# mrmod/h264decode

Hardware: AMD Instinct MI355X
Metric: 1080p Main CABAC frames/sec (higher is better)
Workload: dtype u8; 1 GPU; 1920x1080 Main CABAC IPPP GOP-30, 256 independent streams per GPU (32 distinct, each used 8 times), QP 28, 1 slice/frame, 1 ref; parallelism=streams sharded, no collective

## Files before the change

### h264decode_amd/_lib.py

```python
import ctypes
import os
import re
import subprocess

_HERE = os.path.dirname(os.path.abspath(__file__))
_HEADER = os.path.join(_HERE, "..", "include", "h264mi.h")
_LIBPATH = os.environ.get("H264MI_LIB") or os.path.join(_HERE, "libh264mi.so")

_CT = {"int32_t": ctypes.c_int32, "uint32_t": ctypes.c_uint32, "int64_t": ctypes.c_int64, "uint64_t": ctypes.c_uint64, "uint8_t": ctypes.c_uint8,
       "double": ctypes.c_double, "float": ctypes.c_float, "void": None}


class H264MIError(RuntimeError):
    def __init__(self, code, msg):
        super().__init__("h264mi error %d: %s" % (code, msg))
        self.code = code


def _parse_structs():
    src = open(_HEADER).read()
    src = re.sub(r"/\*.*?\*/", "", src, flags=re.S)
    out = {}
    for body, name in re.findall(r"typedef struct \{(.*?)\}\s*(h264mi_\w+);", src, flags=re.S):
        fields = []
# ... 46 lines not shown
            raise H264MIError(-4, "libh264mi_hooks.so is not built (make -C h264decode_amd/csrc)")
        _hooks = ctypes.CDLL(path)
        I32 = ctypes.c_int32
        _hooks.h264mi_internal_dbprep_kernel_choice.argtypes = [I32, I32]
        _hooks.h264mi_internal_dbprep_kernel_choice.restype = I32
        _hooks.h264mi_internal_dbprep_check.argtypes = [ctypes.c_void_p, ctypes.POINTER(I32), ctypes.POINTER(I32), ctypes.POINTER(ctypes.c_int64)]
        _hooks.h264mi_internal_dbprep_check.restype = I32
        _hooks.h264mi_internal_set_dbprep_rows.argtypes = [ctypes.c_void_p, I32]
        _hooks.h264mi_internal_set_dbprep_rows.restype = I32
        _hooks.h264mi_internal_dbprep_ip_rows.argtypes = [I32, I32, I32]
        _hooks.h264mi_internal_dbprep_ip_rows.restype = I32
        _hooks.h264mi_internal_set_k5_waves.argtypes = [ctypes.c_void_p, I32]
        _hooks.h264mi_internal_set_k5_waves.restype = I32
        _hooks.h264mi_internal_deblock_edge_probe.argtypes = [I32, I32, I32] + [ctypes.c_void_p] * 6 + [ctypes.c_int64]
        _hooks.h264mi_internal_deblock_edge_probe.restype = I32
        _hooks.h264mi_internal_side_pending.argtypes = [ctypes.c_void_p, ctypes.POINTER(I32)]
        _hooks.h264mi_internal_side_pending.restype = I32
    return _hooks


def load():
    global _lib
    if _lib is not None:
        return _lib
    if not os.path.exists(_LIBPATH):
        raise H264MIError(-4, "libh264mi.so is not built (run h264decode_amd.build() / __graft_entry__.build()); "
                              "there is no CPU fallback for the decode path")
    L = ctypes.CDLL(_LIBPATH)
    P, I32, SZ = ctypes.POINTER, ctypes.c_int32, ctypes.c_size_t
    u8p, vp = ctypes.c_char_p, ctypes.c_void_p
# ... 111 lines not shown
```

### h264decode_amd/csrc/k_recon.hip

```cpp
#include <hip/hip_runtime.h>
#include <cstddef>
#include "mi_kernels.h"
#include "k_common.h"
#include "k_residual.h"

__device__ __forceinline__ int clip255(int v) { return min(max(v, 0), 255); }

struct ResBuf {
    int32_t tmp[384];
    int16_t luma[256];
    int16_t chroma[2][64];
    int32_t dc[24];
};

__device__ __forceinline__ void mb_residual(int lane, const MbRec *rec, const int16_t *coef, const ScalingSet *sc, ResBuf *rb) {
    const int type = rec->type, t8x8 = rec->t8x8, cbp = rec->cbp, qp = rec->qp;
    const int intra = MB_IS_INTRA(type), i16 = type == MBT_I16x16;
    const int cbp_l = cbp & 15, cbp_c = cbp >> 4;
    if (i16 && lane < 16) {
        const int i = lane >> 2, j = lane & 3;
        int acc = 0;
#pragma unroll
        for (int k = 0; k < 4; k++) {
            int aik = (i == 0) ? 1 : (i == 1 ? (k < 2 ? 1 : -1) : (i == 2 ? ((k == 0 || k == 3) ? 1 : -1) : ((k & 1) ? -1 : 1)));
            int rowsum = 0;
#pragma unroll
            for (int m = 0; m < 4; m++) {
                int amj = (j == 0) ? 1 : (j == 1 ? (m < 2 ? 1 : -1) : (j == 2 ? ((m == 0 || m == 3) ? 1 : -1) : ((m & 1) ? -1 : 1)));
// ... 93 lines not shown
        int16_t *dst = rb->chroma[c];
        dst[(y0 + 0) * 8 + x0] = static_cast<int16_t>((o0 + 32) >> 6);
        dst[(y0 + 1) * 8 + x0] = static_cast<int16_t>((o1 + 32) >> 6);
        dst[(y0 + 2) * 8 + x0] = static_cast<int16_t>((o2 + 32) >> 6);
        dst[(y0 + 3) * 8 + x0] = static_cast<int16_t>((o3 + 32) >> 6);
    }
    WAVE_SYNC();
}

__device__ __forceinline__ void zero_residual(int lane, ResBuf *rb) {
    for (int i = lane; i < 128; i += 64) reinterpret_cast<uint32_t *>(rb->luma)[i] = 0;
    reinterpret_cast<uint32_t *>(rb->chroma)[lane] = 0;
    WAVE_SYNC();
}

struct IntraWave {
    ResBuf rb;
    uint8_t tile[17][28];
    uint8_t tile_c[2][9][12];
    int16_t fe[2][32];
    MbRec rec;
    alignas(16) int16_t coef[MI_COEF_PER_MB];
};
#define MI_INTRA_MAX_ROWS 320
#define MI_INTRA_MAX_CHUNKS 8
struct IntraShared {
    IntraWave w[MI_INTRA_WAVES];
    ScalingSet sc;
    unsigned long long pend[MI_INTRA_MAX_ROWS][MI_INTRA_MAX_CHUNKS];
};

template <int N, typename FT, typename FL>
__device__ __forceinline__ int pred_dir(int mode, int x, int y, FT T, FL L) {
    switch (mode) {
    case 3: return (x == N - 1 && y == N - 1) ? (T(2 * N - 2) + 3 * T(2 * N - 1) + 2) >> 2 : (T(x + y) + 2 * T(x + y + 1) + T(x + y + 2) + 2) >> 2;
    case 4:
        if (x > y) return (T(x - y - 2) + 2 * T(x - y - 1) + T(x - y) + 2) >> 2;
        if (x < y) return (L(y - x - 2) + 2 * L(y - x - 1) + L(y - x) + 2) >> 2;
        return (T(0) + 2 * T(-1) + L(0) + 2) >> 2;
    case 5: {
        int z = 2 * x - y, k = x - (y >> 1);
        if (z < -1) return (L(y - 2 * x - 1) + 2 * L(y - 2 * x - 2) + L(y - 2 * x - 3) + 2) >> 2;
        if (z == -1) return (L(0) + 2 * T(-1) + T(0) + 2) >> 2;
// ... 9 lines not shown
    }
    case 7: {
        int k = x + (y >> 1);
        return !(y & 1) ? (T(k) + T(k + 1) + 1) >> 1 : (T(k) + 2 * T(k + 1) + T(k + 2) + 2) >> 2;
    }
    default: {
        int z = x + 2 * y, k = y + (x >> 1);
        if (z > 2 * N - 3) return L(N - 1);
        if (z == 2 * N - 3) return (L(N - 2) + 3 * L(N - 1) + 2) >> 2;
        if (!(z & 1)) return (L(k) + L(k + 1) + 1) >> 1;
        return (L(k) + 2 * L(k + 1) + L(k + 2) + 2) >> 2;
    }
    }
}

template <int N, typename FT, typename FL>
__device__ __forceinline__ void plane_params(FT T, FL L, int &a, int &b, int &c) {
    int hh = 0, vv = 0;
    constexpr int m = N / 2;
#pragma unroll
    for (int k = 1; k <= m; k++) {
        hh += k * (T(m - 1 + k) - T(m - 1 - k));
        vv += k * (L(m - 1 + k) - L(m - 1 - k));
    }
    a = 16 * (L(N - 1) + T(N - 1));
    b = N == 16 ? (5 * hh + 32) >> 6 : (34 * hh + 32) >> 6;
    c = N == 16 ? (5 * vv + 32) >> 6 : (34 * vv + 32) >> 6;
}

template <bool X>
__device__ __forceinline__ int ld_px(const g8 *p) {
    if (X) return static_cast<int>(__hip_atomic_load(p, __ATOMIC_RELAXED, __HIP_MEMORY_SCOPE_AGENT));
    return static_cast<int>(*p);
}
template <bool X>
__device__ __forceinline__ void st_px32(g8 *p, uint32_t v) {
    if (X)
        __hip_atomic_store(reinterpret_cast<g32 *>(p), v, __ATOMIC_RELAXED, __HIP_MEMORY_SCOPE_AGENT);
    else
        *reinterpret_cast<g32 *>(p) = v;
}
template <bool X>
__device__ __forceinline__ void st_px16(g8 *p, uint16_t v) {
    if (X)
        __hip_atomic_store(reinterpret_cast<g16 *>(p), v, __ATOMIC_RELAXED, __HIP_MEMORY_SCOPE_AGENT);
    else
        *reinterpret_cast<g16 *>(p) = v;
}

template <bool X>
__device__ void intra_mb(int lane, IntraWave *ws, const MbRec *rec, const int16_t *coef, const ScalingSet *sc, g8 *py, g8 *pcb, g8 *pcr, int W,
                         int mbx, int mby) {
    const int type = rec->type, av = rec->avail;
    const int a_left = av & MI_AV_LEFT, a_top = (av & MI_AV_TOP) != 0, a_tl = (av & MI_AV_TOPLEFT) != 0, a_tr = (av & MI_AV_TOPRIGHT) != 0;
    g8 *Y = py + static_cast<size_t>(mby * 16) * W + mbx * 16;
    const int Wc = W / 2;
    g8 *C0 = pcb + static_cast<size_t>(mby * 8) * Wc + mbx * 8, *C1 = pcr + static_cast<size_t>(mby * 8) * Wc + mbx * 8;
#define CPL(c) ((c) ? C1 : C0)
    if (type == MBT_NONE) {
        st_px32<X>(Y + static_cast<size_t>(lane >> 2) * W + (lane & 3) * 4, 0x80808080u);
        if (lane < 32) st_px32<X>(CPL(lane >> 4) + static_cast<size_t>((lane >> 1) & 7) * Wc + (lane & 1) * 4, 0x80808080u);
        return;
    }
    if (type == MBT_IPCM) {
        const uint8_t *pcm = reinterpret_cast<const uint8_t *>(coef);
        {
            int j = lane >> 2, i = (lane & 3) * 4;
// ... 13 lines not shown
        int y = lane - 32;
        ws->tile[y + 1][0] = a_left ? static_cast<uint8_t>(ld_px<X>(Y + static_cast<size_t>(y) * W - 1)) : static_cast<uint8_t>(128);
    }
    if (lane < 18) {
        int c = lane / 9, x = lane % 9 - 1;
        int ok = x < 0 ? a_tl : a_top;
        ws->tile_c[c][0][x + 1] = ok ? static_cast<uint8_t>(ld_px<X>(CPL(c) - static_cast<ptrdiff_t>(Wc) + x)) : static_cast<uint8_t>(128);
    } else if (lane >= 32 && lane < 48) {
        int c = (lane - 32) >> 3, y = lane & 7;
        ws->tile_c[c][y + 1][0] = a_left ? static_cast<uint8_t>(ld_px<X>(CPL(c) + static_cast<size_t>(y) * Wc - 1)) : static_cast<uint8_t>(128);
    }
    if ((rec->cbp & 0x3F) || type == MBT_I16x16)
        mb_residual(lane, rec, coef, sc, &ws->rb);
    else
        zero_residual(lane, &ws->rb);
    if (type == MBT_I16x16) {
        const int mode = rec->i16mode;
        auto T = [&](int x) { return static_cast<int>(ws->tile[0][x + 1]); };
        auto L = [&](int y) { return static_cast<int>(ws->tile[y + 1][0]); };
        const int j = lane >> 2, i0 = (lane & 3) * 4;
        int dc = 128, pa = 0, pb = 0, pc = 0;
        if (mode == 2) {
            int st = 0, sl = 0;
#pragma unroll
            for (int k = 0; k < 16; k++) st += T(k), sl += L(k);
            if (a_top && a_left)
                dc = (st + sl + 16) >> 5;
            else if (a_top)
                dc = (st + 8) >> 4;
            else if (a_left)
                dc = (sl + 8) >> 4;
        } else if (mode == 3)
            plane_params<16>(T, L, pa, pb, pc);
        uint32_t packed = 0;
#pragma unroll
        for (int k = 0; k < 4; k++) {
            int x = i0 + k, v;
            if (mode == 0)
                v = T(x);
            else if (mode == 1)
                v = L(j);
            else if (mode == 2)
                v = dc;
            else
                v = clip255((pa + pb * (x - 7) + pc * (j - 7) + 16) >> 5);
            v = clip255(v + ws->rb.luma[j * 16 + x]);
            packed |= static_cast<uint32_t>(v) << (8 * k);
        }
        st_px32<X>(Y + static_cast<size_t>(j) * W + i0, packed);
    } else if (type == MBT_I4x4) {
        for (int d = 0; d < 10; d++) {
            const int half = lane >> 4;
            const int by = (d >= 2 && d <= 7) ? (d & 1 ? (half ? 1 + ((d - 3) >> 1) : (d - 3) >> 1) : (half ? (d >> 1) : (d >> 1) - 1)) : (d < 2 ? 0 : 3);
            const int bx = d - 2 * by;
            const bool two = d >= 2 && d <= 7;
            if (lane < (two ? 32 : 16)) {
                const int mode = rec->ipm[by * 4 + bx];
                const int has_left = bx > 0 || a_left, has_top = by > 0 || a_top;
                int has_tr;
                if (by == 0)
                    has_tr = bx < 3 ? a_top : a_tr;
                else
                    has_tr = bx == 3 ? 0 : !((bx & 1) && (by & 1));
                const int x = lane & 3, y = (lane >> 2) & 3;
                const uint8_t *trow = &ws->tile[by * 4][bx * 4 + 1];
                auto T = [&](int k) { return static_cast<int>((k >= 4 && !has_tr) ? trow[3] : trow[k]); };
                auto L = [&](int k) { return k < 0 ? static_cast<int>(trow[-1]) : static_cast<int>(ws->tile[by * 4 + 1 + k][bx * 4]); };
                int v;
                if (mode == 0)
                    v = T(x);
                else if (mode == 1)
                    v = L(y);
                else if (mode == 2) {
                    int st = T(0) + T(1) + T(2) + T(3), sl = L(0) + L(1) + L(2) + L(3);
                    v = (has_top && has_left) ? (st + sl + 4) >> 3 : (has_top ? (st + 2) >> 2 : (has_left ? (sl + 2) >> 2 : 128));
                } else
                    v = pred_dir<4>(mode, x, y, T, L);
                v = clip255(v + ws->rb.luma[(by * 4 + y) * 16 + bx * 4 + x]);
                ws->tile[by * 4 + 1 + y][bx * 4 + 1 + x] = static_cast<uint8_t>(v);
            }
            WAVE_SYNC();
        }
    } else {
        for (int b8 = 0; b8 < 4; b8++) {
            const int x8 = b8 & 1, y8 = b8 >> 1;
            const int mode = rec->ipm[y8 * 8 + x8 * 2];
            const int has_left = x8 || a_left, has_top = y8 || a_top;
            const int has_tl = b8 == 0 ? a_tl : (b8 == 1 ? a_top : (b8 == 2 ? (a_left != 0) : 1));
            const int has_tr = b8 == 0 ? a_top : (b8 == 1 ? a_tr : (b8 == 2 ? 1 : 0));
            const uint8_t *trow = &ws->tile[y8 * 8][x8 * 8 + 1];
            auto Tr = [&](int k) { return k < 0 ? static_cast<int>(trow[-1]) : static_cast<int>((k >= 8 && !has_tr) ? trow[7] : trow[k]); };
            auto Lr = [&](int k) { return k < 0 ? static_cast<int>(trow[-1]) : static_cast<int>(ws->tile[y8 * 8 + 1 + k][x8 * 8]); };
            if (lane < 17) {
                int x = lane - 1, v;
                if (x < 0) {
                    if (has_top && has_left)
                        v = (Tr(0) + 2 * Tr(-1) + Lr(0) + 2) >> 2;
// ... 32 lines not shown
                    v = L(y);
                else if (mode == 2) {
                    int st = 0, sl = 0;
#pragma unroll
                    for (int k = 0; k < 8; k++) st += T(k), sl += L(k);
                    v = (has_top && has_left) ? (st + sl + 8) >> 4 : (has_top ? (st + 4) >> 3 : (has_left ? (sl + 4) >> 3 : 128));
                } else
                    v = pred_dir<8>(mode, x, y, T, L);
                v = clip255(v + ws->rb.luma[(y8 * 8 + y) * 16 + x8 * 8 + x]);
                WAVE_SYNC();
                ws->tile[y8 * 8 + 1 + y][x8 * 8 + 1 + x] = static_cast<uint8_t>(v);
            }
            WAVE_SYNC();
        }
    }
    if (type != MBT_I16x16) {
        const int j = lane >> 2, i0 = (lane & 3) * 4;
        const uint8_t *t = &ws->tile[j + 1][i0 + 1];
        uint32_t packed = t[0] | (t[1] << 8) | (t[2] << 16) | (static_cast<uint32_t>(t[3]) << 24);
        st_px32<X>(Y + static_cast<size_t>(j) * W + i0, packed);
    }
    {
        const int mode = rec->chroma_mode;
        const int c = lane >> 5, q = lane & 31, y = q >> 2, x0 = (q & 3) * 2;
        auto T = [&](int k) { return static_cast<int>(ws->tile_c[c][0][k + 1]); };
        auto L = [&](int k) { return static_cast<int>(ws->tile_c[c][k + 1][0]); };
        int pa = 0, pb = 0, pc = 0, dc = 128;
        if (mode == 3)
            plane_params<8>(T, L, pa, pb, pc);
        else if (mode == 0) {
            const int xo = x0 & 4, yo = y & 4;
            int st = T(xo) + T(xo + 1) + T(xo + 2) + T(xo + 3), sl = L(yo) + L(yo + 1) + L(yo + 2) + L(yo + 3);
            int use_t = a_top, use_l = a_left != 0;
            if (xo && !yo && a_top)
                use_l = 0;
            else if (!xo && yo && a_left)
                use_t = 0;
            if (use_t && use_l)
                dc = (st + sl + 4) >> 3;
            else if (use_t)
                dc = (st + 2) >> 2;
            else if (use_l)
                dc = (sl + 2) >> 2;
        }
        uint32_t packed = 0;
#pragma unroll
        for (int k = 0; k < 2; k++) {
            int x = x0 + k, v;
            if (mode == 0)
                v = dc;
            else if (mode == 1)
                v = L(y);
            else if (mode == 2)
                v = T(x);
            else
                v = clip255((pa + pb * (x - 3) + pc * (y - 3) + 16) >> 5);
            v = clip255(v + ws->rb.chroma[c][y * 8 + x]);
            packed |= static_cast<uint32_t>(v) << (8 * k);
        }
        st_px16<X>(CPL(c) + static_cast<size_t>(y) * Wc + x0, static_cast<uint16_t>(packed));
    }
}


struct IntraPic {
    int wmb, hmb, nchunks;
    int W;
    g8 *py, *pcb, *pcr;
    uint64_t mb_base;
    const MbRec *recs;
    __device__ __forceinline__ IntraPic(const PicDesc *pd, const DevTables *tab, const MbRec *mbrec, ScalingSet *sc, int tid, int nthreads) {
        wmb = static_cast<int>(pd->wmb), hmb = static_cast<int>(pd->hmb);
        W = static_cast<int>(pd->pitch);
        const PicPlace pp(pd);
        py = pp.base + pp.y, pcb = pp.base + pp.cb, pcr = pp.base + pp.cr;
        const uint32_t *src = reinterpret_cast<const uint32_t *>(&tab->scaling[pd->scaling_set]);
        for (int i = tid; i < static_cast<int>(sizeof(ScalingSet) / 4); i += nthreads) reinterpret_cast<uint32_t *>(sc)[i] = src[i];
        nchunks = (wmb + 63) >> 6;
        mb_base = pd->mb_base, recs = mbrec + mb_base;
    }
};

__device__ __forceinline__ unsigned long long intra_bits(const unsigned long long *mask, unsigned long long first, int n) {
    const unsigned long long w = first >> 6;
    const int sh = static_cast<int>(first & 63);
    unsigned long long m = mask[w] >> sh;
    if (sh) m |= mask[w + 1] << (64 - sh);
    return n >= 64 ? m : (m & ((1ull << n) - 1ull));
}

typedef unsigned long long IntraRows[MI_INTRA_MAX_ROWS][MI_INTRA_MAX_CHUNKS];

// ... 42 lines not shown
    if (ln < MI_COEF_BLOCKS) reinterpret_cast<uint4 *>(ws->coef)[2 * ln] = c0, reinterpret_cast<uint4 *>(ws->coef)[2 * ln + 1] = c1;
    WAVE_SYNC();
}

__device__ __forceinline__ void mb_done(IntraShared *sh, int mbx, int mby, int ln) {
    if (ln == 0) __hip_atomic_fetch_and(&sh->pend[mby][mbx >> 6], ~(1ull << (mbx & 63)), __ATOMIC_RELEASE, __HIP_MEMORY_SCOPE_WORKGROUP);
}

extern "C" __global__ void __launch_bounds__(MI_INTRA_WAVES * 64) k_intra(const uint32_t *pic_list, const PicDesc *pics, const FramePool *pools, const DevTables *tab,
                                                                          const MbRec *mbrec, const int16_t *coefs, const unsigned long long *intramask) {
    __shared__ IntraShared sh;
    __shared__ IntraRows s_intra;
    __shared__ uint32_t s_prefix[MI_INTRA_MAX_ROWS + 1];
    __shared__ uint32_t s_next;
    const int tid = static_cast<int>(threadIdx.x), lane = tid & 63, wave = tid >> 6;
    const IntraPic ip(&pics[pic_list[blockIdx.x]], tab, mbrec, &sh.sc, tid, MI_INTRA_WAVES * 64);
    const int wmb = ip.wmb, hmb = ip.hmb, nchunks = ip.nchunks;
    load_intra_masks(ip, intramask, &sh, s_intra, 0, hmb, tid, MI_INTRA_WAVES * 64);
    if (tid == 0) s_next = 0;
    __syncthreads();
    if (tid == 0) {
        uint32_t acc = 0;
        s_prefix[0] = 0;
        for (int r = 0; r < hmb; r++) {
            for (int c = 0; c < nchunks; c++) acc += static_cast<uint32_t>(__builtin_popcountll(s_intra[r][c]));
            s_prefix[r + 1] = acc;
        }
    }
    __syncthreads();
    IntraWave *ws = &sh.w[wave];
    const uint32_t n_intra = s_prefix[hmb];
// ... 27 lines not shown
                if (++chunk == nchunks) chunk = 0, row += MI_INTRA_WAVES;
                if (row >= hmb) break;
                mask = s_intra[row][chunk];
            }
            if (!mask) break;
            mbx = chunk * 64 + __ffsll(static_cast<long long>(mask)) - 1, mby = row;
            mask &= mask - 1;
        }
        mbx = __builtin_amdgcn_readfirstlane(mbx), mby = __builtin_amdgcn_readfirstlane(mby);
        int ln = lane;
        OPAQUE(ln);
        load_rec(ws, ip.recs + static_cast<uint64_t>(mby) * wmb + mbx, ln);
        if (sparse && mbx > 0) wait_mb(&sh, mbx - 1, mby);
        if (mby > 0) wait_row_above(&sh, mby, AboveSpan(mbx, wmb));
        gather_coefs(ws, coefs, ln);
        intra_mb<false>(ln, ws, &ws->rec, ws->coef, &sh.sc, ip.py, ip.pcb, ip.pcr, ip.W, mbx, mby);
        mb_done(&sh, mbx, mby, ln);
    }
}

extern "C" __global__ void __launch_bounds__(MI_INTRA_WAVES * 64) k_intra_x(const uint32_t *pic_list, const PicDesc *pics, const FramePool *pools, const DevTables *tab,
                                                                            const MbRec *mbrec, const int16_t *coefs, uint32_t *xdone_, uint32_t epoch, int nbands,
                                                                            uint32_t *ticket, uint32_t ticket_base, int wmb_max, uint32_t *xstatus, int wpr,
                                                                            const unsigned long long *intramask) {
    __shared__ IntraShared sh;
    __shared__ IntraRows s_intra;
    __shared__ uint32_t s_ticket;
    const int tid = static_cast<int>(threadIdx.x), lane = tid & 63, wave = tid >> 6, nthreads = static_cast<int>(blockDim.x), nwaves = nthreads >> 6;
    if (tid == 0) s_ticket = atomicAdd(ticket, 1u) - ticket_base;
    __syncthreads();
    const uint32_t tk = s_ticket, pic_i = tk / static_cast<uint32_t>(nbands);
    const int band = static_cast<int>(tk - pic_i * static_cast<uint32_t>(nbands));
    const PicDesc *pd = &pics[pic_list[pic_i]];
    const int wmb = static_cast<int>(pd->wmb), hmb = static_cast<int>(pd->hmb);
    const int r0 = band * hmb / nbands, r1 = (band + 1) * hmb / nbands;
    if (r0 >= r1) return;
    const IntraPic ip(pd, tab, mbrec, &sh.sc, tid, nthreads);
    const int nchunks = ip.nchunks;
    typedef __attribute__((address_space(1))) uint32_t gflag;
    int pband = band - 1;
    while (pband > 0 && pband * hmb / nbands == (pband + 1) * hmb / nbands) pband--;
    gflag *const xin = (gflag *)xdone_ + (static_cast<size_t>(pic_i) * nbands + (pband > 0 ? pband : 0)) * static_cast<size_t>(wmb_max);
    gflag *const xout = (gflag *)xdone_ + (static_cast<size_t>(pic_i) * nbands + band) * static_cast<size_t>(wmb_max);
    load_intra_masks(ip, intramask, &sh, s_intra, r0 > 0 ? r0 - 1 : 0, r1, tid, nthreads);
    __syncthreads();
    IntraWave *ws = &sh.w[wave];
    const int row_slot = wave / wpr, turn = wave - row_slot * wpr, row_slots = nwaves / wpr;
    for (int mby = r0 + row_slot; mby < r1; mby += row_slots) {
        const MbRec *row = ip.recs + static_cast<uint64_t>(mby) * wmb;
        const bool publish = mby == r1 - 1 && r1 < hmb;
        int nth = 0;
        for (int c = 0; c < nchunks; c++) {
// ... 16 lines not shown
                        const bool need = ln < 3 && col <= up.xr && ((sh.pend[mby - 1][col >> 6] >> (col & 63)) & 1ull);
                        const unsigned long long t_start = __builtin_amdgcn_s_memrealtime();
                        for (;;) {
                            const uint32_t v = need ? __hip_atomic_load(xin + col, __ATOMIC_RELAXED, __HIP_MEMORY_SCOPE_AGENT) : epoch;
                            if (__builtin_amdgcn_ballot_w64(v != epoch) == 0) break;
                            __builtin_amdgcn_s_sleep(2);
                            if (__builtin_amdgcn_s_memrealtime() - t_start > 400000000ull) {
                                if (ln == 0) atomicExch(xstatus, 0x3D000000u | static_cast<uint32_t>(mby));
                                break;
                            }
                        }
                        __builtin_amdgcn_fence(__ATOMIC_ACQUIRE, "wavefront");
                    }
                }
                gather_coefs(ws, coefs, ln);
                intra_mb<true>(ln, ws, &ws->rec, ws->coef, &sh.sc, ip.py, ip.pcb, ip.pcr, ip.W, mbx, mby);
                if (publish) {
                    asm volatile("s_waitcnt vmcnt(0)" ::: "memory");
                    if (ln == 0) __hip_atomic_store(xout + mbx, epoch, __ATOMIC_RELAXED, __HIP_MEMORY_SCOPE_AGENT);
                }
                mb_done(&sh, mbx, mby, ln);
            }
        }
    }
}
```

### h264decode_amd/csrc/mi_hooks.cpp

```cpp
#include <hip/hip_runtime.h>
#include <algorithm>
#include <cstdio>
#include <cstdlib>
#include <vector>
#include "mi_decoder.hpp"
#if defined(H264MI_TEST_HOOKS) && defined(__HIP__)
#include "k_deblock_edge.h"
#include "k_deblock_pk.h"
#endif

#if !defined(H264MI_TEST_HOOKS)
void hook_create_entropy(h264mi_decoder *, int *) {}
void hook_create_k5(h264mi_decoder *) {}
int hook_entropy_kernel(int chosen) { return chosen; }
int hook_dbprep_kernel(int chosen) { return chosen; }
void hook_after_sync(const h264mi_decoder *) {}
#else
void hook_create_entropy(h264mi_decoder *d, int *ent_cus) {
    if (const char *e = getenv("H264MI_ENT_LDS_PAD")) d->ent_lds_pad = static_cast<size_t>(atoi(e));
    if (const char *e = getenv("H264MI_ENT_CUS")) *ent_cus = atoi(e);
}
void hook_create_k5(h264mi_decoder *d) {
    if (const char *e = getenv("H264MI_K5_WAVES")) d->k5_max_waves = std::min(std::max(atoi(e), 1), MI_DEBLOCK8_MAX_WAVES);
}
// ... 261 lines not shown
    int nb = 1, nw = 1, ring = 1, b3 = 1, w3 = 1, roles = 1;
    mi_deblock_bands(n_pics, wmb, hmb, max_wgs, &nb, &nw, &ring, &roles);
    int wpr = 1;
    mi_intra_bands(n_pics, hmb, max_wgs, false, &b3, &w3, &wpr);
    *k5_bands = nb, *k5_waves = nw / roles, *k5_ring = ring, *k5_lds = static_cast<int64_t>(mi_deblock_lds_bytes_banded(nw, ring));
    *k3_bands = b3, *k3_waves = w3;
    return H264MI_OK;
}

extern "C" int32_t h264mi_internal_intra_plan(int32_t n_pics, int32_t hmb, int32_t max_wgs, int32_t p_only, int32_t band, int32_t *bands, int32_t *waves, int32_t *wpr, int32_t *row0) {
    if (!bands || !waves || !wpr || !row0 || n_pics < 1 || hmb < 1 || band < 0) return H264MI_EINVAL;
    int nb = 1, nw = 1, w = 1;
    mi_intra_bands(n_pics, hmb, max_wgs, p_only != 0, &nb, &nw, &w);
    *bands = nb, *waves = nw, *wpr = w, *row0 = band < nb ? band * hmb / nb : hmb;
    return H264MI_OK;
}

extern "C" int32_t h264mi_internal_set_epoch(h264mi_decoder *d, uint32_t v) {
    if (!d) return H264MI_EINVAL;
    GUARD(d);
    if (const int r = drain(d)) return r;
    d->x_epoch = d->x_tk5 = d->x_tk3 = v;
    HIP_TRY(hipMemcpy(d->d_xctl, &d->x_tk5, sizeof(uint32_t), hipMemcpyHostToDevice));
    HIP_TRY(hipMemcpy(d->d_xctl + 32, &d->x_tk3, sizeof(uint32_t), hipMemcpyHostToDevice));
    return H264MI_OK;
}

extern "C" int32_t h264mi_internal_dpb_trace(h264mi_decoder *d, int32_t stream, char *buf, size_t cap, size_t *len) {
    if (!d || !buf || !len || !cap || stream < 0 || stream >= static_cast<int>(d->st.size())) return H264MI_EINVAL;
    const Stage &g = d->stage[d->prep];
// ... 97 lines not shown
```

Measured before the change: 30350 frames/s.

## Rewrite intra prediction with lane-parallel DPP reductions and 4x4 pick table

Replaces the per-lane serial intra prediction (loops over edge samples for DC/plane, per-mode formulas) with cross-lane DPP/bpermute reductions for 16x16 and chroma DC/plane. It also adds a constexpr lookup table that maps each 4x4 mode/pixel to one of four precomputed edge vectors (edge, 3-tap, 2-tap, DC). Several 4x4 blocks are predicted in parallel along diagonals. The goal is to cut instruction count and divergence in the intra reconstruction kernel, at the cost of more LDS for the table and more complex lane shuffles. Test probes are added to check the new paths.

```diff
diff --git a/h264decode_amd/_lib.py b/h264decode_amd/_lib.py
--- a/h264decode_amd/_lib.py
+++ b/h264decode_amd/_lib.py
@@ -84,6 +84,10 @@
         _hooks.h264mi_internal_set_k5_waves.restype = I32
         _hooks.h264mi_internal_deblock_edge_probe.argtypes = [I32, I32, I32] + [ctypes.c_void_p] * 6 + [ctypes.c_int64]
         _hooks.h264mi_internal_deblock_edge_probe.restype = I32
+        _hooks.h264mi_internal_intra_pick_table.argtypes = [I32, ctypes.c_void_p, ctypes.c_int64]
+        _hooks.h264mi_internal_intra_pick_table.restype = I32
+        _hooks.h264mi_internal_intra_block_probe.argtypes = [I32] + [ctypes.c_void_p] * 5 + [ctypes.c_int64]
+        _hooks.h264mi_internal_intra_block_probe.restype = I32
         _hooks.h264mi_internal_side_pending.argtypes = [ctypes.c_void_p, ctypes.POINTER(I32)]
         _hooks.h264mi_internal_side_pending.restype = I32
     return _hooks
diff --git a/h264decode_amd/csrc/k_intra_pred.h b/h264decode_amd/csrc/k_intra_pred.h
--- /dev/null
+++ b/h264decode_amd/csrc/k_intra_pred.h
@@ -0,0 +1,239 @@
+#pragma once
+#include <hip/hip_runtime.h>
+#include <cstddef>
+#include <cstdint>
+#include "mi_kernels.h"
+#include "k_common.h"
+
+enum { IP_E = 0, IP_F3 = 1, IP_F2 = 2, IP_DC = 3 };
+#define IP4_LINE 13
+#define IP_BAD 0xFF
+constexpr uint8_t ip_pick(int vec, int idx) { return (idx < 0 || idx > 15) ? IP_BAD : static_cast<uint8_t>(idx << 2 | vec); }
+constexpr int ip4_t(int k) { return 5 + k; }
+constexpr int ip4_l(int k) { return 3 - k; }
+constexpr uint8_t ip4_tap3(int p, int q, int r) {
+    const int lo = p < r ? p : r, hi = p < r ? r : p;
+    const bool inner = lo == q - 1 && hi == q + 1, low_end = q == 0 && lo == 0 && hi == 1, high_end = q == IP4_LINE - 1 && lo == q - 1 && hi == q;
+    return (inner || low_end || high_end) ? ip_pick(IP_F3, q) : static_cast<uint8_t>(IP_BAD);
+}
+constexpr uint8_t ip4_tap2(int p, int q) { return (p - q == 1 || q - p == 1) ? ip_pick(IP_F2, p < q ? p : q) : static_cast<uint8_t>(IP_BAD); }
+constexpr uint8_t ip4_entry(int mode, int x, int y) {
+    switch (mode) {
+    case 0: return ip_pick(IP_E, ip4_t(x));
+    case 1: return ip_pick(IP_E, ip4_l(y));
+    case 2: return ip_pick(IP_DC, 0);
+    case 3: return (x == 3 && y == 3) ? ip4_tap3(ip4_t(6), ip4_t(7), ip4_t(7)) : ip4_tap3(ip4_t(x + y), ip4_t(x + y + 1), ip4_t(x + y + 2));
+    case 4:
+        if (x > y) return ip4_tap3(ip4_t(x - y - 2), ip4_t(x - y - 1), ip4_t(x - y));
+        if (x < y) return ip4_tap3(ip4_l(y - x - 2), ip4_l(y - x - 1), ip4_l(y - x));
+        return ip4_tap3(ip4_t(0), ip4_t(-1), ip4_l(0));
+    case 5: {
+        const int z = 2 * x - y, k = x - (y >> 1);
+        if (z < -1) return ip4_tap3(ip4_l(y - 2 * x - 1), ip4_l(y - 2 * x - 2), ip4_l(y - 2 * x - 3));
+        if (z == -1) return ip4_tap3(ip4_l(0), ip4_t(-1), ip4_t(0));
+        if (!(z & 1)) return ip4_tap2(ip4_t(k - 1), ip4_t(k));
+        return ip4_tap3(ip4_t(k - 2), ip4_t(k - 1), ip4_t(k));
+    }
+    case 6: {
+        const int z = 2 * y - x, k = y - (x >> 1);
+        if (z < -1) return ip4_tap3(ip4_t(x - 2 * y - 1), ip4_t(x - 2 * y - 2), ip4_t(x - 2 * y - 3));
+        if (z == -1) return ip4_tap3(ip4_l(0), ip4_t(-1), ip4_t(0));
+        if (!(z & 1)) return ip4_tap2(ip4_l(k - 1), ip4_l(k));
+        return ip4_tap3(ip4_l(k - 2), ip4_l(k - 1), ip4_l(k));
+    }
+    case 7: {
+        const int k = x + (y >> 1);
+        return !(y & 1) ? ip4_tap2(ip4_t(k), ip4_t(k + 1)) : ip4_tap3(ip4_t(k), ip4_t(k + 1), ip4_t(k + 2));
+    }
+    default: {
+        const int z = x + 2 * y, k = y + (x >> 1);
+        if (z > 5) return ip_pick(IP_E, ip4_l(3));
+        if (z == 5) return ip4_tap3(ip4_l(2), ip4_l(3), ip4_l(3));
+        if (!(z & 1)) return ip4_tap2(ip4_l(k), ip4_l(k + 1));
+        return ip4_tap3(ip4_l(k), ip4_l(k + 1), ip4_l(k + 2));
+    }
+    }
+}
+struct alignas(16) Ip4Table {
+    uint8_t e[9 * 16];
+};
+constexpr Ip4Table ip4_make_table() {
+    Ip4Table t{};
+    for (int m = 0; m < 9; m++)
+        for (int i = 0; i < 16; i++) t.e[m * 16 + i] = ip4_entry(m, i & 3, i >> 2);
+    return t;
+}
+constexpr bool ip4_table_ok(const Ip4Table &t) {
+    for (int i = 0; i < 9 * 16; i++)
+        if (t.e[i] == IP_BAD) return false;
+    return true;
+}
+constexpr Ip4Table ip4_table = ip4_make_table();
+static_assert(ip4_table_ok(ip4_table), "a formula of 8.3.1.2 that is no pick from E / F3 / F2 / DC");
+
+#if defined(__HIP__)
+static __constant__ Ip4Table ip4_table_dev = ip4_make_table();
+
+__device__ __forceinline__ int clip255(int v) { return min(max(v, 0), 255); }
+
+struct ResBuf {
+    int32_t tmp[384];
+    int16_t luma[256];
+    int16_t chroma[2][64];
+    int32_t dc[24];
+};
+#define IP_TILE_PITCH 28
+struct IntraWave {
+    ResBuf rb;
+    uint8_t tile[17][IP_TILE_PITCH];
+    uint8_t tile_c[2][9][12];
+    int16_t fe[2][32];
+    MbRec rec;
+    alignas(16) int16_t coef[MI_COEF_PER_MB];
+};
+
+template <bool X>
+__device__ __forceinline__ int ld_px(const g8 *p) {
+    if (X) return static_cast<int>(__hip_atomic_load(p, __ATOMIC_RELAXED, __HIP_MEMORY_SCOPE_AGENT));
+    return static_cast<int>(*p);
+}
+template <bool X>
+__device__ __forceinline__ void st_px32(g8 *p, uint32_t v) {
+    if (X)
+        __hip_atomic_store(reinterpret_cast<g32 *>(p), v, __ATOMIC_RELAXED, __HIP_MEMORY_SCOPE_AGENT);
+    else
+        *reinterpret_cast<g32 *>(p) = v;
+}
+template <bool X>
+__device__ __forceinline__ void st_px16(g8 *p, uint16_t v) {
+    if (X)
+        __hip_atomic_store(reinterpret_cast<g16 *>(p), v, __ATOMIC_RELAXED, __HIP_MEMORY_SCOPE_AGENT);
+    else
+        *reinterpret_cast<g16 *>(p) = v;
+}
+
+#define IP_DPP_QUAD_1032 0xB1
+#define IP_DPP_QUAD_2301 0x4E
+#define IP_DPP_ROW_SHL1 0x101
+#define IP_DPP_ROW_SHR1 0x111
+#define IP_DPP_ROW_ROR(n) (0x120 + (n))
+#define IP_DPP_HALF_MIRROR 0x141
+template <int CTRL>
+__device__ __forceinline__ int ip_row_nb(int v) { return __builtin_amdgcn_update_dpp(v, v, CTRL, 0xF, 0xF, false); }
+template <int CTRL>
+__device__ __forceinline__ int ip_dpp(int v) { return __builtin_amdgcn_update_dpp(0, v, CTRL, 0xF, 0xF, false); }
+__device__ __forceinline__ int ip_row_sum(int v) {
+    v += ip_dpp<IP_DPP_ROW_ROR(8)>(v);
+    v += ip_dpp<IP_DPP_ROW_ROR(4)>(v);
+    v += ip_dpp<IP_DPP_ROW_ROR(2)>(v);
+    v += ip_dpp<IP_DPP_ROW_ROR(1)>(v);
+    return v;
+}
+__device__ __forceinline__ int ip_quad_sum(int v) {
+    v += ip_dpp<IP_DPP_QUAD_1032>(v);
+    v += ip_dpp<IP_DPP_QUAD_2301>(v);
+    return v;
+}
+__device__ __forceinline__ int ip_lane_get(int v, int src_lane) { return __builtin_amdgcn_ds_bpermute(src_lane << 2, v); }
+
+__device__ __forceinline__ int ip4_sample(const uint8_t *corner, int lane, int pick, int res, int has_left, int has_top, int has_tr) {
+    const int l = lane & 15;
+    int k = min(l - 4, 8);
+    k = (k >= 5 && !has_tr) ? 4 : k;
+    const int e = corner[l < 4 ? (4 - l) * IP_TILE_PITCH : k];
+    const int below = ip_row_nb<IP_DPP_ROW_SHR1>(e), above = ip_row_nb<IP_DPP_ROW_SHL1>(e);
+    const int f3 = (below + 2 * e + above + 2) >> 2, f2 = (e + above + 1) >> 1;
+    const int s = ip_row_sum((l < 4 ? e : 0) | ((l >= 5 && l < 9) ? e << 16 : 0));
+    const int st = has_top ? s >> 16 : 0, sl = has_left ? s & 0xFFFF : 0, n = (has_top != 0) + (has_left != 0);
+    const int dc = n ? (st + sl + (1 << n)) >> (n + 1) : 128;
+    const uint32_t vecs = static_cast<uint32_t>(e) | static_cast<uint32_t>(f3) << 8 | static_cast<uint32_t>(f2) << 16 | static_cast<uint32_t>(dc) << 24;
+    const uint32_t got = static_cast<uint32_t>(__builtin_amdgcn_ds_bpermute(((lane & 0x30) << 2) | (pick & 0x3C), static_cast<int>(vecs)));
+    const int pred = static_cast<int>((got >> ((pick & 3) << 3)) & 255u);
+    return clip255(pred + res);
+}
+
+template <bool X>
+__device__ __forceinline__ void ip16_luma(int lane, const IntraWave *ws, int mode, int a_top, int a_left, g8 *Y, int W) {
+    const uint8_t *tile = &ws->tile[0][0];
+    const int j = lane >> 2, i0 = (lane & 3) * 4;
+    int p0, p1, p2, p3;
+    if (mode == 0) {
+        const uint32_t *row = reinterpret_cast<const uint32_t *>(tile + i0);
+        unpack4(__builtin_amdgcn_alignbyte(row[1], row[0], 1), p0, p1, p2, p3);
+    } else if (mode == 1)
+        p0 = p1 = p2 = p3 = tile[(j + 1) * IP_TILE_PITCH];
+    else {
+        const int r = lane & 31, i = r & 15, plane = mode == 3;
+        const int e = tile[(plane && i == 7) ? 0 : (r < 16 ? i + 1 : (i + 1) * IP_TILE_PITCH)];
+        const int s = ip_row_sum(plane ? (i == 7 ? -8 : i - 7) * e : e);
+        const int top = __builtin_amdgcn_readlane(s, 0), left = __builtin_amdgcn_readlane(s, 16);
+        if (!plane) {
+            int dc = 128;
+            if (a_top && a_left)
+                dc = (top + left + 16) >> 5;
+            else if (a_top)
+                dc = (top + 8) >> 4;
+            else if (a_left)
+                dc = (left + 8) >> 4;
+            p0 = p1 = p2 = p3 = dc;
+        } else {
+            const int a = 16 * (__builtin_amdgcn_readlane(e, 15) + __builtin_amdgcn_readlane(e, 31));
+            const int b = (5 * top + 32) >> 6, c = (5 * left + 32) >> 6;
+            const int base = a + b * (i0 - 7) + c * (j - 7) + 16;
+            p0 = clip255(base >> 5), p1 = clip255((base + b) >> 5), p2 = clip255((base + 2 * b) >> 5), p3 = clip255((base + 3 * b) >> 5);
+        }
+    }
+    const v2u rr = *reinterpret_cast<const v2u *>(&ws->rb.luma[j * 16 + i0]);
+    const int r0 = static_cast<int16_t>(rr.x & 0xFFFFu), r1 = static_cast<int>(rr.x) >> 16, r2 = static_cast<int16_t>(rr.y & 0xFFFFu), r3 = static_cast<int>(rr.y) >> 16;
+    st_px32<X>(Y + static_cast<size_t>(j) * W + i0, pack4(clip255(p0 + r0), clip255(p1 + r1), clip255(p2 + r2), clip255(p3 + r3)));
+}
+
+template <bool X>
+__device__ __forceinline__ void ip_tile_to_frame(int lane, const IntraWave *ws, g8 *Y, int W) {
+    const int j = lane >> 2, i0 = (lane & 3) * 4;
+    const uint32_t *row = reinterpret_cast<const uint32_t *>(&ws->tile[j + 1][i0]);
+    st_px32<X>(Y + static_cast<size_t>(j) * W + i0, __builtin_amdgcn_alignbyte(row[1], row[0], 1));
+}
+
+template <bool X>
+__device__ __forceinline__ void ip_chroma(int lane, const IntraWave *ws, int mode, int a_top, int a_left, g8 *C, int Wc) {
+    const int c = lane >> 5, q = lane & 31, y = q >> 2, x0 = (q & 3) * 2, first = lane & 32;
+    const uint8_t *tile = &ws->tile_c[c][0][0];
+    int p0, p1;
+    if (mode == 1)
+        p0 = p1 = tile[(y + 1) * 12];
+    else if (mode == 2)
+        p0 = tile[x0 + 1], p1 = tile[x0 + 2];
+    else {
+        const int i = q & 7, plane = mode == 3;
+        const int e = tile[(plane && i == 3) ? 0 : ((q & 8) ? (i + 1) * 12 : i + 1)];
+        if (!plane) {
+            const int s = ip_quad_sum(e), xo = x0 & 4, yo = y & 4;
+            const int st = ip_lane_get(s, first + xo), sl = ip_lane_get(s, first + 8 + yo);
+            int use_t = a_top, use_l = a_left != 0, dc = 128;
+            if (xo && !yo && a_top)
+                use_l = 0;
+            else if (!xo && yo && a_left)
+                use_t = 0;
+            if (use_t && use_l)
+                dc = (st + sl + 4) >> 3;
+            else if (use_t)
+                dc = (st + 2) >> 2;
+            else if (use_l)
+                dc = (sl + 2) >> 2;
+            p0 = p1 = dc;
+        } else {
+            int s = ip_quad_sum((i == 3 ? -4 : i - 3) * e);
+            s += ip_dpp<IP_DPP_HALF_MIRROR>(s);
+            const int hh = ip_lane_get(s, first), vv = ip_lane_get(s, first + 8);
+            const int a = 16 * (ip_lane_get(e, first + 7) + ip_lane_get(e, first + 15));
+            const int b = (34 * hh + 32) >> 6, cc = (34 * vv + 32) >> 6;
+            const int base = a + b * (x0 - 3) + cc * (y - 3) + 16;
+            p0 = clip255(base >> 5), p1 = clip255((base + b) >> 5);
+        }
+    }
+    const uint32_t rr = *reinterpret_cast<const uint32_t *>(&ws->rb.chroma[c][y * 8 + x0]);
+    const int r0 = static_cast<int16_t>(rr & 0xFFFFu), r1 = static_cast<int>(rr) >> 16;
+    st_px16<X>(C + static_cast<size_t>(y) * Wc + x0, static_cast<uint16_t>(clip255(p0 + r0) | clip255(p1 + r1) << 8));
+}
+#endif
diff --git a/h264decode_amd/csrc/k_recon.hip b/h264decode_amd/csrc/k_recon.hip
--- a/h264decode_amd/csrc/k_recon.hip
+++ b/h264decode_amd/csrc/k_recon.hip
@@ -3,15 +3,7 @@
 #include "mi_kernels.h"
 #include "k_common.h"
 #include "k_residual.h"
-
-__device__ __forceinline__ int clip255(int v) { return min(max(v, 0), 255); }
-
-struct ResBuf {
-    int32_t tmp[384];
-    int16_t luma[256];
-    int16_t chroma[2][64];
-    int32_t dc[24];
-};
+#include "k_intra_pred.h"
 
 __device__ __forceinline__ void mb_residual(int lane, const MbRec *rec, const int16_t *coef, const ScalingSet *sc, ResBuf *rb) {
     const int type = rec->type, t8x8 = rec->t8x8, cbp = rec->cbp, qp = rec->qp;
@@ -135,19 +127,12 @@
     WAVE_SYNC();
 }
 
-struct IntraWave {
-    ResBuf rb;
-    uint8_t tile[17][28];
-    uint8_t tile_c[2][9][12];
-    int16_t fe[2][32];
-    MbRec rec;
-    alignas(16) int16_t coef[MI_COEF_PER_MB];
-};
 #define MI_INTRA_MAX_ROWS 320
 #define MI_INTRA_MAX_CHUNKS 8
 struct IntraShared {
     IntraWave w[MI_INTRA_WAVES];
     ScalingSet sc;
+    Ip4Table pick4;
     unsigned long long pend[MI_INTRA_MAX_ROWS][MI_INTRA_MAX_CHUNKS];
 };
 
@@ -187,43 +172,9 @@
     }
 }
 
-template <int N, typename FT, typename FL>
-__device__ __forceinline__ void plane_params(FT T, FL L, int &a, int &b, int &c) {
-    int hh = 0, vv = 0;
-    constexpr int m = N / 2;
-#pragma unroll
-    for (int k = 1; k <= m; k++) {
-        hh += k * (T(m - 1 + k) - T(m - 1 - k));
-        vv += k * (L(m - 1 + k) - L(m - 1 - k));
-    }
-    a = 16 * (L(N - 1) + T(N - 1));
-    b = N == 16 ? (5 * hh + 32) >> 6 : (34 * hh + 32) >> 6;
-    c = N == 16 ? (5 * vv + 32) >> 6 : (34 * vv + 32) >> 6;
-}
-
 template <bool X>
-__device__ __forceinline__ int ld_px(const g8 *p) {
-    if (X) return static_cast<int>(__hip_atomic_load(p, __ATOMIC_RELAXED, __HIP_MEMORY_SCOPE_AGENT));
-    return static_cast<int>(*p);
-}
-template <bool X>
-__device__ __forceinline__ void st_px32(g8 *p, uint32_t v) {
-    if (X)
-        __hip_atomic_store(reinterpret_cast<g32 *>(p), v, __ATOMIC_RELAXED, __HIP_MEMORY_SCOPE_AGENT);
-    else
-        *reinterpret_cast<g32 *>(p) = v;
-}
-template <bool X>
-__device__ __forceinline__ void st_px16(g8 *p, uint16_t v) {
-    if (X)
-        __hip_atomic_store(reinterpret_cast<g16 *>(p), v, __ATOMIC_RELAXED, __HIP_MEMORY_SCOPE_AGENT);
-    else
-        *reinterpret_cast<g16 *>(p) = v;
-}
-
-template <bool X>
-__device__ void intra_mb(int lane, IntraWave *ws, const MbRec *rec, const int16_t *coef, const ScalingSet *sc, g8 *py, g8 *pcb, g8 *pcr, int W,
-                         int mbx, int mby) {
+__device__ void intra_mb(int lane, IntraWave *ws, const MbRec *rec, const int16_t *coef, const ScalingSet *sc, const Ip4Table *pk, g8 *py, g8 *pcb, g8 *pcr,
+                         int W, int mbx, int mby) {
     const int type = rec->type, av = rec->avail;
     const int a_left = av & MI_AV_LEFT, a_top = (av & MI_AV_TOP) != 0, a_tl = (av & MI_AV_TOPLEFT) != 0, a_tr = (av & MI_AV_TOPRIGHT) != 0;
     g8 *Y = py + static_cast<size_t>(mby * 16) * W + mbx * 16;
@@ -267,73 +218,34 @@
         mb_residual(lane, rec, coef, sc, &ws->rb);
     else
         zero_residual(lane, &ws->rb);
-    if (type == MBT_I16x16) {
-        const int mode = rec->i16mode;
-        auto T = [&](int x) { return static_cast<int>(ws->tile[0][x + 1]); };
-        auto L = [&](int y) { return static_cast<int>(ws->tile[y + 1][0]); };
-        const int j = lane >> 2, i0 = (lane & 3) * 4;
-        int dc = 128, pa = 0, pb = 0, pc = 0;
-        if (mode == 2) {
-            int st = 0, sl = 0;
-#pragma unroll
-            for (int k = 0; k < 16; k++) st += T(k), sl += L(k);
-            if (a_top && a_left)
-                dc = (st + sl + 16) >> 5;
-            else if (a_top)
-                dc = (st + 8) >> 4;
-            else if (a_left)
-                dc = (sl + 8) >> 4;
-        } else if (mode == 3)
-            plane_params<16>(T, L, pa, pb, pc);
-        uint32_t packed = 0;
-#pragma unroll
-        for (int k = 0; k < 4; k++) {
-            int x = i0 + k, v;
-            if (mode == 0)
-                v = T(x);
-            else if (mode == 1)
-                v = L(j);
-            else if (mode == 2)
-                v = dc;
+    if (type == MBT_I16x16)
+        ip16_luma<X>(lane, ws, rec->i16mode, a_top, a_left, Y, W);
+    else if (type == MBT_I4x4) {
+        const int half = (lane >> 4) & 1, l = lane & 15, x = l & 3, y = l >> 2;
+#define I4_BY(d) (((d) >= 2 && (d) <= 7) ? ((d) & 1 ? (half ? 1 + (((d) - 3) >> 1) : ((d) - 3) >> 1) : (half ? ((d) >> 1) : ((d) >> 1) - 1)) : ((d) < 2 ? 0 : 3))
+        int pick[10], res[10];
+#pragma unroll
+        for (int d = 0; d < 10; d++) {
+            const int by = I4_BY(d), bx = d - 2 * by;
+            pick[d] = pk->e[min(max(static_cast<int>(rec->ipm[by * 4 + bx]), 0), 8) * 16 + l];
+            res[d] = ws->rb.luma[(by * 4 + y) * 16 + bx * 4 + x];
+        }
+#pragma unroll
+        for (int d = 0; d < 10; d++) {
+            const int by = I4_BY(d), bx = d - 2 * by;
+            const bool two = d >= 2 && d <= 7;
+            const int has_left = bx > 0 || a_left, has_top = by > 0 || a_top;
+            int has_tr;
+            if (by == 0)
+                has_tr = bx < 3 ? a_top : a_tr;
             else
-                v = clip255((pa + pb * (x - 7) + pc * (j - 7) + 16) >> 5);
-            v = clip255(v + ws->rb.luma[j * 16 + x]);
-            packed |= static_cast<uint32_t>(v) << (8 * k);
-        }
-        st_px32<X>(Y + static_cast<size_t>(j) * W + i0, packed);
-    } else if (type == MBT_I4x4) {
-        for (int d = 0; d < 10; d++) {
-            const int half = lane >> 4;
-            const int by = (d >= 2 && d <= 7) ? (d & 1 ? (half ? 1 + ((d - 3) >> 1) : (d - 3) >> 1) : (half ? (d >> 1) : (d >> 1) - 1)) : (d < 2 ? 0 : 3);
-            const int bx = d - 2 * by;
-            const bool two = d >= 2 && d <= 7;
-            if (lane < (two ? 32 : 16)) {
-                const int mode = rec->ipm[by * 4 + bx];
-                const int has_left = bx > 0 || a_left, has_top = by > 0 || a_top;
-                int has_tr;
-                if (by == 0)
-                    has_tr = bx < 3 ? a_top : a_tr;
-                else
-                    has_tr = bx == 3 ? 0 : !((bx & 1) && (by & 1));
-                const int x = lane & 3, y = (lane >> 2) & 3;
-                const uint8_t *trow = &ws->tile[by * 4][bx * 4 + 1];
-                auto T = [&](int k) { return static_cast<int>((k >= 4 && !has_tr) ? trow[3] : trow[k]); };
-                auto L = [&](int k) { return k < 0 ? static_cast<int>(trow[-1]) : static_cast<int>(ws->tile[by * 4 + 1 + k][bx * 4]); };
-                int v;
-                if (mode == 0)
-                    v = T(x);
-                else if (mode == 1)
-                    v = L(y);
-                else if (mode == 2) {
-                    int st = T(0) + T(1) + T(2) + T(3), sl = L(0) + L(1) + L(2) + L(3);
-                    v = (has_top && has_left) ? (st + sl + 4) >> 3 : (has_top ? (st + 2) >> 2 : (has_left ? (sl + 2) >> 2 : 128));
-                } else
-                    v = pred_dir<4>(mode, x, y, T, L);
-                v = clip255(v + ws->rb.luma[(by * 4 + y) * 16 + bx * 4 + x]);
-                ws->tile[by * 4 + 1 + y][bx * 4 + 1 + x] = static_cast<uint8_t>(v);
-            }
+                has_tr = bx == 3 ? 0 : !((bx & 1) && (by & 1));
+            uint8_t *corner = &ws->tile[by * 4][bx * 4];
+            const int v = ip4_sample(corner, lane, pick[d], res[d], has_left, has_top, has_tr);
+            if (lane < (two ? 32 : 16)) corner[(1 + y) * IP_TILE_PITCH + 1 + x] = static_cast<uint8_t>(v);
             WAVE_SYNC();
         }
+#undef I4_BY
     } else {
         for (int b8 = 0; b8 < 4; b8++) {
             const int x8 = b8 & 1, y8 = b8 >> 1;
@@ -396,52 +308,8 @@
             WAVE_SYNC();
         }
     }
-    if (type != MBT_I16x16) {
-        const int j = lane >> 2, i0 = (lane & 3) * 4;
-        const uint8_t *t = &ws->tile[j + 1][i0 + 1];
-        uint32_t packed = t[0] | (t[1] << 8) | (t[2] << 16) | (static_cast<uint32_t>(t[3]) << 24);
-        st_px32<X>(Y + static_cast<size_t>(j) * W + i0, packed);
-    }
-    {
-        const int mode = rec->chroma_mode;
-        const int c = lane >> 5, q = lane & 31, y = q >> 2, x0 = (q & 3) * 2;
-        auto T = [&](int k) { return static_cast<int>(ws->tile_c[c][0][k + 1]); };
-        auto L = [&](int k) { return static_cast<int>(ws->tile_c[c][k + 1][0]); };
-        int pa = 0, pb = 0, pc = 0, dc = 128;
-        if (mode == 3)
-            plane_params<8>(T, L, pa, pb, pc);
-        else if (mode == 0) {
-            const int xo = x0 & 4, yo = y & 4;
-            int st = T(xo) + T(xo + 1) + T(xo + 2) + T(xo + 3), sl = L(yo) + L(yo + 1) + L(yo + 2) + L(yo + 3);
-            int use_t = a_top, use_l = a_left != 0;
-            if (xo && !yo && a_top)
-                use_l = 0;
-            else if (!xo && yo && a_left)
-                use_t = 0;
-            if (use_t && use_l)
-                dc = (st + sl + 4) >> 3;
-            else if (use_t)
-                dc = (st + 2) >> 2;
-            else if (use_l)
-                dc = (sl + 2) >> 2;
-        }
-        uint32_t packed = 0;
-#pragma unroll
-        for (int k = 0; k < 2; k++) {
-            int x = x0 + k, v;
-            if (mode == 0)
-                v = dc;
-            else if (mode == 1)
-                v = L(y);
-            else if (mode == 2)
-                v = T(x);
-            else
-                v = clip255((pa + pb * (x - 3) + pc * (y - 3) + 16) >> 5);
-            v = clip255(v + ws->rb.chroma[c][y * 8 + x]);
-            packed |= static_cast<uint32_t>(v) << (8 * k);
-        }
-        st_px16<X>(CPL(c) + static_cast<size_t>(y) * Wc + x0, static_cast<uint16_t>(packed));
-    }
+    if (type != MBT_I16x16) ip_tile_to_frame<X>(lane, ws, Y, W);
+    ip_chroma<X>(lane, ws, rec->chroma_mode, a_top, a_left, CPL(lane >> 5), Wc);
 }
 
 
@@ -451,13 +319,14 @@
     g8 *py, *pcb, *pcr;
     uint64_t mb_base;
     const MbRec *recs;
-    __device__ __forceinline__ IntraPic(const PicDesc *pd, const DevTables *tab, const MbRec *mbrec, ScalingSet *sc, int tid, int nthreads) {
+    __device__ __forceinline__ IntraPic(const PicDesc *pd, const DevTables *tab, const MbRec *mbrec, ScalingSet *sc, Ip4Table *pick4, int tid, int nthreads) {
         wmb = static_cast<int>(pd->wmb), hmb = static_cast<int>(pd->hmb);
         W = static_cast<int>(pd->pitch);
         const PicPlace pp(pd);
         py = pp.base + pp.y, pcb = pp.base + pp.cb, pcr = pp.base + pp.cr;
         const uint32_t *src = reinterpret_cast<const uint32_t *>(&tab->scaling[pd->scaling_set]);
         for (int i = tid; i < static_cast<int>(sizeof(ScalingSet) / 4); i += nthreads) reinterpret_cast<uint32_t *>(sc)[i] = src[i];
+        for (int i = tid; i < static_cast<int>(sizeof(Ip4Table) / 4); i += nthreads) reinterpret_cast<uint32_t *>(pick4)[i] = reinterpret_cast<const uint32_t *>(&ip4_table_dev)[i];
         nchunks = (wmb + 63) >> 6;
         mb_base = pd->mb_base, recs = mbrec + mb_base;
     }
@@ -530,7 +399,7 @@
     __shared__ uint32_t s_prefix[MI_INTRA_MAX_ROWS + 1];
     __shared__ uint32_t s_next;
     const int tid = static_cast<int>(threadIdx.x), lane = tid & 63, wave = tid >> 6;
-    const IntraPic ip(&pics[pic_list[blockIdx.x]], tab, mbrec, &sh.sc, tid, MI_INTRA_WAVES * 64);
+    const IntraPic ip(&pics[pic_list[blockIdx.x]], tab, mbrec, &sh.sc, &sh.pick4, tid, MI_INTRA_WAVES * 64);
     const int wmb = ip.wmb, hmb = ip.hmb, nchunks = ip.nchunks;
     load_intra_masks(ip, intramask, &sh, s_intra, 0, hmb, tid, MI_INTRA_WAVES * 64);
     if (tid == 0) s_next = 0;
@@ -588,7 +457,7 @@
         if (sparse && mbx > 0) wait_mb(&sh, mbx - 1, mby);
         if (mby > 0) wait_row_above(&sh, mby, AboveSpan(mbx, wmb));
         gather_coefs(ws, coefs, ln);
-        intra_mb<false>(ln, ws, &ws->rec, ws->coef, &sh.sc, ip.py, ip.pcb, ip.pcr, ip.W, mbx, mby);
+        intra_mb<false>(ln, ws, &ws->rec, ws->coef, &sh.sc, &sh.pick4, ip.py, ip.pcb, ip.pcr, ip.W, mbx, mby);
         mb_done(&sh, mbx, mby, ln);
     }
 }
@@ -609,7 +478,7 @@
     const int wmb = static_cast<int>(pd->wmb), hmb = static_cast<int>(pd->hmb);
     const int r0 = band * hmb / nbands, r1 = (band + 1) * hmb / nbands;
     if (r0 >= r1) return;
-    const IntraPic ip(pd, tab, mbrec, &sh.sc, tid, nthreads);
+    const IntraPic ip(pd, tab, mbrec, &sh.sc, &sh.pick4, tid, nthreads);
     const int nchunks = ip.nchunks;
     typedef __attribute__((address_space(1))) uint32_t gflag;
     int pband = band - 1;
@@ -656,7 +525,7 @@
                     }
                 }
                 gather_coefs(ws, coefs, ln);
-                intra_mb<true>(ln, ws, &ws->rec, ws->coef, &sh.sc, ip.py, ip.pcb, ip.pcr, ip.W, mbx, mby);
+                intra_mb<true>(ln, ws, &ws->rec, ws->coef, &sh.sc, &sh.pick4, ip.py, ip.pcb, ip.pcr, ip.W, mbx, mby);
                 if (publish) {
                     asm volatile("s_waitcnt vmcnt(0)" ::: "memory");
                     if (ln == 0) __hip_atomic_store(xout + mbx, epoch, __ATOMIC_RELAXED, __HIP_MEMORY_SCOPE_AGENT);
diff --git a/h264decode_amd/csrc/mi_hooks.cpp b/h264decode_amd/csrc/mi_hooks.cpp
--- a/h264decode_amd/csrc/mi_hooks.cpp
+++ b/h264decode_amd/csrc/mi_hooks.cpp
@@ -7,6 +7,7 @@
 #if defined(H264MI_TEST_HOOKS) && defined(__HIP__)
 #include "k_deblock_edge.h"
 #include "k_deblock_pk.h"
+#include "k_intra_pred.h"
 #endif
 
 #if !defined(H264MI_TEST_HOOKS)
@@ -299,6 +300,91 @@
     mi_intra_bands(n_pics, hmb, max_wgs, p_only != 0, &nb, &nw, &w);
     *bands = nb, *waves = nw, *wpr = w, *row0 = band < nb ? band * hmb / nb : hmb;
     return H264MI_OK;
+}
+
+extern "C" int32_t h264mi_internal_intra_pick_table(int32_t n, uint8_t *out, int64_t cap) {
+#if defined(__HIP__)
+    if (!out || n != 4 || cap < static_cast<int64_t>(sizeof(ip4_table.e))) return H264MI_EINVAL;
+    std::copy(ip4_table.e, ip4_table.e + sizeof(ip4_table.e), out);
+    return static_cast<int32_t>(sizeof(ip4_table.e));
+#else
+    set_error("h264mi_internal_intra_pick_table: this build holds no device code");
+    return H264MI_ENODEVICE;
+#endif
+}
+
+#if defined(__HIP__)
+__global__ void __launch_bounds__(64) k_ip_probe4(const uint8_t *mode, const uint8_t *comb, const uint8_t *edge, const int16_t *res, uint8_t *out) {
+    __shared__ uint8_t tiles[4][5 * IP_TILE_PITCH];
+    __shared__ Ip4Table pk;
+    const int lane = static_cast<int>(threadIdx.x), l = lane & 15;
+    const size_t blk = static_cast<size_t>(blockIdx.x) * 4 + (lane >> 4);
+    if (lane < static_cast<int>(sizeof(Ip4Table) / 4)) reinterpret_cast<uint32_t *>(&pk)[lane] = reinterpret_cast<const uint32_t *>(&ip4_table_dev)[lane];
+    uint8_t *corner = tiles[lane >> 4];
+    if (l < IP4_LINE) corner[l < 4 ? (4 - l) * IP_TILE_PITCH : l - 4] = edge[blk * IP4_LINE + l];
+    __syncthreads();
+    const int cb = comb[blk];
+    const int v = ip4_sample(corner, lane, pk.e[mode[blk] * 16 + l], res[blk * 16 + l], cb & 1, cb & 2, cb & 8);
+    out[blk * 16 + l] = static_cast<uint8_t>(v);
+}
+__global__ void __launch_bounds__(64) k_ip_probe16(const uint8_t *mode, const uint8_t *comb, const uint8_t *edge, const int16_t *res, uint8_t *out) {
+    __shared__ IntraWave ws;
+    const int lane = static_cast<int>(threadIdx.x);
+    const size_t blk = blockIdx.x;
+    if (lane < 33) ws.tile[lane < 16 ? 16 - lane : 0][lane < 16 ? 0 : lane - 16] = edge[blk * 33 + lane];
+    for (int i = lane; i < 256; i += 64) ws.rb.luma[i] = res[blk * 256 + i];
+    __syncthreads();
+    const int cb = comb[blk];
+    ip16_luma<false>(lane, &ws, mode[blk], (cb & 2) != 0, cb & 1, (g8 *)(out + blk * 256), 16);
+}
+__global__ void __launch_bounds__(64) k_ip_probe_c(const uint8_t *mode, const uint8_t *comb, const uint8_t *edge, const int16_t *res, uint8_t *out) {
+    __shared__ IntraWave ws;
+    const int lane = static_cast<int>(threadIdx.x);
+    const size_t blk = blockIdx.x;
+    if (lane < 34) {
+        const int c = lane / 17, i = lane % 17;
+        ws.tile_c[c][i < 8 ? 8 - i : 0][i < 8 ? 0 : i - 8] = edge[blk * 34 + lane];
+    }
+    for (int i = lane; i < 128; i += 64) ws.rb.chroma[i >> 6][i & 63] = res[blk * 128 + i];
+    __syncthreads();
+    const int cb = comb[blk];
+    ip_chroma<false>(lane, &ws, mode[blk], (cb & 2) != 0, cb & 1, (g8 *)(out + blk * 128 + (lane >> 5) * 64), 8);
+}
+#endif
+extern "C" int32_t h264mi_internal_intra_block_probe(int32_t kind, const uint8_t *mode, const uint8_t *comb, const uint8_t *edge, const int16_t *res, uint8_t *out, int64_t n) {
+    if (!mode || !comb || !edge || !res || !out || kind < 0 || kind > 2 || n < 4 || n % 4 != 0 || n > (int64_t(1) << 18)) return H264MI_EINVAL;
+    for (int64_t i = 0; i < n; i++)
+        if (mode[i] > (kind == 0 ? 8 : 3) || comb[i] > 15) return H264MI_EINVAL;
+#if defined(__HIP__)
+    const size_t un = static_cast<size_t>(n), line = kind == 0 ? IP4_LINE : (kind == 1 ? 33 : 34), px = kind == 0 ? 16 : (kind == 1 ? 256 : 128);
+    uint8_t *dev = nullptr;
+    hipError_t e = hipMalloc(&dev, un * (3 * px + line + 2));
+    uint8_t *d_r = dev, *d_o = dev + un * 2 * px, *d_e = d_o + un * px, *d_m = d_e + un * line, *d_c = d_m + un;
+    if (e == hipSuccess) e = hipMemcpy(d_r, res, un * 2 * px, hipMemcpyHostToDevice);
+    if (e == hipSuccess) e = hipMemset(d_o, 0xA5, un * px);
+    if (e == hipSuccess) e = hipMemcpy(d_e, edge, un * line, hipMemcpyHostToDevice);
+    if (e == hipSuccess) e = hipMemcpy(d_m, mode, un, hipMemcpyHostToDevice);
+    if (e == hipSuccess) e = hipMemcpy(d_c, comb, un, hipMemcpyHostToDevice);
+    if (e == hipSuccess) {
+        const dim3 grid(static_cast<uint32_t>(kind == 0 ? un / 4 : un)), block(64);
+        const int16_t *d_r16 = reinterpret_cast<const int16_t *>(d_r);
+        if (kind == 0) hipLaunchKernelGGL(k_ip_probe4, grid, block, 0, 0, d_m, d_c, d_e, d_r16, d_o);
+        else if (kind == 1) hipLaunchKernelGGL(k_ip_probe16, grid, block, 0, 0, d_m, d_c, d_e, d_r16, d_o);
+        else hipLaunchKernelGGL(k_ip_probe_c, grid, block, 0, 0, d_m, d_c, d_e, d_r16, d_o);
+        e = hipGetLastError();
+    }
+    if (e == hipSuccess) e = hipDeviceSynchronize();
+    if (e == hipSuccess) e = hipMemcpy(out, d_o, un * px, hipMemcpyDeviceToHost);
+    if (dev) hipFree(dev);
+    if (e != hipSuccess) {
+        set_error("h264mi_internal_intra_block_probe failed: %s", hipGetErrorString(e));
+        return H264MI_EDEVICE;
+    }
+    return H264MI_OK;
+#else
+    set_error("h264mi_internal_intra_block_probe: this build holds no device code");
+    return H264MI_ENODEVICE;
+#endif
 }
 
 extern "C" int32_t h264mi_internal_set_epoch(h264mi_decoder *d, uint32_t v) {
```

New measurement: 30630 frames/s, median of 6. Within noise of the previous version (+0.9%).
